# IceTTTb/NopeSAC

Hardware: AMD Instinct MI355X
Metric: image-pairs/sec (480x640, K=32 hyp) (higher is better)
Workload: dtype bf16; 1 GPU; configs/inference_mp3d.yaml, 32 synthetic 480x640 pairs/GPU/step, ResNet-50 + pyramids in bfloat16, head GEMMs bf16 operands with f32 accumulate / residual stream / LayerNorm / softmax, K=32 matched planes forced (m mean 32.0), nq=50; pairs_per_gpu=32, global_batch=32, K=32, parallelism=pair-sharded dp1, rccl_ranks=1, batches_in_flight_per_gpu=4, hip_graph=False, steps_per_all_gather=8, routing_entries_loaded=45, routing_entries_measured_now=0, nonfinite_outputs=0

## Files before the change

### include/nopesac_hip.h

```cpp
#ifndef NOPESAC_HIP_H
#define NOPESAC_HIP_H

#include <stdint.h>

#ifdef __cplusplus
extern "C" {
#endif

#define NPS_DT_F32 0
#define NPS_DT_BF16 1
#define NPS_DT_F32_BF16W 2
#define NPS_DT_FP8 3

#define NPS_ACT_NONE 0
#define NPS_ACT_RELU 1
#define NPS_ACT_LEAKY 2
#define NPS_ACT_SIGMOID 3
#define NPS_ACT_RES_AFTER 0x100
#define NPS_ACT_BIAS_BATCHED 0x200

#define NPS_E_ARG (-1)
#define NPS_E_UNSUPPORTED (-2)

int nopesac_version(void);
// ... 18 lines not shown

int nopesac_conv2d_nhwc_bfrag(const void* x, const void* w_frag, const float* scale, const float* bias, const void* residual,
                              void* y, int B, int H, int W, int Cin, int Cout, int KH, int KW, int stride, int pad,
                              int64_t x_cstride, int64_t y_cstride, int64_t r_cstride, int act, int out_dt, int variant,
                              void* stream);

int nopesac_conv2d_nhwc_p8(const void* x, const void* w, const float* scale, const float* bias, const void* residual, void* y,
                           int B, int H, int W, int Cin, int Cout, int KH, int KW, int stride, int pad,
                           int64_t x_cstride, int64_t y_cstride, int64_t r_cstride, int act, int out_dt, int variant, void* stream);

int64_t nopesac_conv2d_p8_sk_workspace_bytes(void);
int nopesac_conv2d_nhwc_p8_sk(const void* x, const void* w, const float* scale, const float* bias, const void* residual, void* y,
                              int B, int H, int W, int Cin, int Cout, int KH, int KW, int stride, int pad,
                              int64_t x_cstride, int64_t y_cstride, int64_t r_cstride, int act, int out_dt, int variant,
                              void* workspace, int64_t workspace_bytes, void* stream);

int nopesac_conv2d_nhwc_p8n(const void* x, const void* w, const float* scale, const float* bias, void* y, int B, int H, int W,
                            int Cin, int Cout, int KH, int KW, int stride, int pad, int64_t x_cstride, int64_t y_cstride, int act,
                            int variant, void* stream);
int nopesac_conv2d_nhwc_p8n_splitk(const void* x, const void* w, const float* scale, const float* bias, void* y, int B, int H, int W,
                                   int Cin, int Cout, int KH, int KW, int stride, int pad, int64_t x_cstride, int64_t y_cstride, int act,
                                   int variant, int splits, void* workspace, int64_t workspace_bytes, void* stream);

#define NOPESAC_MLP_MAX_IN 1280
#define NOPESAC_MLP_MAX_WIDTH 1024
#define NOPESAC_MLP_MAX_LAYERS 12
#define NOPESAC_MLP_RESTART 1
typedef struct nopesac_mlp_layer {
    const void* w;
    const float* bias;
    float* out;
    int64_t out_ld;
    int K, N, act, reserved;
} nopesac_mlp_layer;
typedef struct nopesac_mlp_chain {
    const float* x;
    int64_t x_ld;
    const float* xb;
    int64_t xb_ld;
    int x_width, xb_width, xb_rows_per, rows, n_layers, reserved;
    nopesac_mlp_layer layers[NOPESAC_MLP_MAX_LAYERS];
} nopesac_mlp_chain;
int nopesac_mlp_padded_k(int N, int K);
int64_t nopesac_mlp_packed_elems(int N, int K);
int nopesac_mlp_chain_bf16(const nopesac_mlp_chain* chain, void* stream);

int nopesac_conv2d_nhwc_fp8(const void* x, const void* w_frag8, const float* scale, const float* bias, const void* residual,
                            void* y, int B, int H, int W, int Cin, int Cout, int KH, int KW, int stride, int pad,
                            int64_t x_cstride, int64_t y_cstride, int64_t r_cstride, int act, int out_dt, int variant,
                            void* stream);

int nopesac_conv3x3_c64_bf16(const void* x, const void* w_frag, const float* scale, const float* bias, void* y, int B, int H, int W,
                             int act, void* stream);

int nopesac_conv3x3_halo_bf16(const void* x, const void* w_frag, const float* scale, const float* bias, void* y, int B, int H, int W,
                              int Cin, int Cout, int act, int tile, void* stream);

int nopesac_stem_fused_bf16(const void* x, const void* w, const float* scale, const float* bias, void* y,
                            int B, int H, int W, void* stream);
int nopesac_stem_fused_raw_bf16(const float* x_nchw, const float* mean, const float* std, const void* w, const float* scale,
                                const float* bias, void* y, int B, int H, int W, void* stream);
int nopesac_stem_fused_raw_shifted_bf16(const float* x_nchw, const float* pad3, const void* w_folded, const float* scale,
                                        const float* bias_folded, void* y, int B, int H, int W, void* stream);

int nopesac_bottleneck_tail_bf16(const void* b, const void* w3, const float* scale3, const float* bias3, const void* residual,
                                 const void* x2, const void* wsc, const float* scale_sc, const float* bias_sc, int B, int OH, int OW,
                                 int x2_H, int x2_W, int x2_stride, int C, int C4, int C2, void* y, const void* w1,
                                 const float* scale1, const float* bias1, int CN, void* o, void* stream);
int nopesac_bottleneck_tail_bf16_ex(const void* b, const void* w3, const float* scale3, const float* bias3, const void* residual,
                                    const void* x2, const void* wsc, const float* scale_sc, const float* bias_sc, int B, int OH, int OW,
                                    int x2_H, int x2_W, int x2_stride, int C, int C4, int C2, void* y, const void* w1,
                                    const float* scale1, const float* bias1, int CN, void* o, int o_dt, void* stream);

int nopesac_preprocess_nchw_to_nhwc(const float* x, void* y, const float* mean, const float* std,
                                    int B, int C, int H, int W, int Cpad, int out_dt, void* stream);

int nopesac_maxpool_nhwc(const void* x, void* y, int B, int H, int W, int C, int K, int stride, int pad,
                         int dt, void* stream);

int nopesac_upsample2x_bilinear_nhwc(const void* x, const void* addend, void* y, int B, int H, int W, int C,
                                     int act, int dt, void* stream);
int nopesac_upsample2x_nearest_add_nhwc(const void* x, const void* lateral, void* y, int B, int H, int W,
                                        int C, int dt, void* stream);

int nopesac_groupnorm_nhwc(const void* x, const float* gamma, const float* beta, void* y,
                           int B, int HW, int C, int G, float eps, int act, int dt, float* workspace, void* stream);

int nopesac_layernorm(const float* x, const float* res, const float* gamma, const float* beta,
                      float* y, const float* addend, int addend_rows, float* y2,
                      int rows, int D, float eps, void* stream);

int nopesac_layernorm_ex(const float* x, const float* res, const float* gamma, const float* beta,
                         float* y, const float* addend, int addend_rows, float* y2, void* y_bf16, void* y2_bf16,
                         int rows, int D, float eps, void* stream);

int nopesac_add_rows(const float* a, const float* b, float* out, int rows, int D, int b_rows, void* stream);

int nopesac_metric_rows(const float* trans, const float* rot, const int32_t* n1, const int32_t* n2, const int32_t* m,
                        const float* t_err, const float* r_err, const int32_t* nonfinite, int pair_idx0, float* rows, int B, void* stream);

int nopesac_concat_cols(const float* a, int Da, const float* b, int Db, float* out, int rows, void* stream);

int nopesac_add_rows_bf16(const float* a, const float* b, void* a_bf16, void* ab_bf16, int rows, int D, int b_rows, void* stream);

int nopesac_softmax_rows(const float* x, float* y, int rows, int D, void* stream);

// ... 234 lines not shown
```

### nopesac_amd/_lib.py

```python
from __future__ import annotations

import ctypes
import os
import re
from ctypes import c_char_p, c_float, c_int, c_int64, c_void_p

HERE = os.path.dirname(os.path.abspath(__file__))
LIB_PATH = os.path.join(HERE, "libnopesac_hip.so")
HEADER_PATH = os.path.join(os.path.dirname(HERE), "include", "nopesac_hip.h")

P, I, L, F = c_void_p, c_int, c_int64, c_float

SIGNATURES = {
    "nopesac_version": [],
    "nopesac_last_error": [],
    "nopesac_conv2d_nhwc": [P, P, P, P, P, P, I, I, I, I, I, I, I, I, I, L, L, L, L, I, I, I, P],
    "nopesac_conv2d_nhwc_bfrag": [P, P, P, P, P, P, I, I, I, I, I, I, I, I, I, L, L, L, I, I, I, P],
    "nopesac_conv2d_nhwc_p8": [P, P, P, P, P, P, I, I, I, I, I, I, I, I, I, L, L, L, I, I, I, P],
    "nopesac_conv2d_nhwc_p8_sk": [P, P, P, P, P, P, I, I, I, I, I, I, I, I, I, L, L, L, I, I, I, P, L, P],
    "nopesac_conv2d_p8_sk_workspace_bytes": [],
    "nopesac_conv2d_nhwc_p8n": [P, P, P, P, P, I, I, I, I, I, I, I, I, I, L, L, I, I, P],
    "nopesac_conv2d_nhwc_p8n_splitk": [P, P, P, P, P, I, I, I, I, I, I, I, I, I, L, L, I, I, I, P, L, P],
    "nopesac_conv2d_nhwc_ex": [P, P, P, P, P, P, I, I, I, I, I, I, I, I, I, L, L, L, L, I, I, I, I, P],
    "nopesac_stem_fused_bf16": [P, P, P, P, P, I, I, I, P],
    "nopesac_stem_fused_raw_bf16": [P, P, P, P, P, P, P, I, I, I, P],
    "nopesac_stem_fused_raw_shifted_bf16": [P, P, P, P, P, P, I, I, I, P],
    "nopesac_bottleneck_tail_bf16": [P] * 9 + [I] * 9 + [P] * 4 + [I, P, P],
    "nopesac_bottleneck_tail_bf16_ex": [P] * 9 + [I] * 9 + [P] * 4 + [I, P, I, P],
    "nopesac_conv2d_nhwc_fp8": [P, P, P, P, P, P, I, I, I, I, I, I, I, I, I, L, L, L, I, I, I, P],
    "nopesac_gnn_layer_bf16": [P, I, P, I, P, I, I, I, P, P] + [P] * 10 + [P],
    "nopesac_gnn_layer_bf16_pf": [P, I, P, I, P, I, I, I, P, P] + [P] * 10 + [P, I, P],
    "nopesac_encoder_tail_bf16": [P] * 13 + [I] + [P] * 3 + [I, P],
    "nopesac_resize_bilinear_u8": [P, I, I, I, P, I, I, P],
    "nopesac_resize_bilinear_u8_batch": [P, I, L, I, I, I, P, I, I, I, P],
    "nopesac_mask_head_bf16": [P] * 9 + [I] * 5 + [P],
    "nopesac_mask_operands": [P, I, P, P, I, I, I, P],
    "nopesac_decoder_tail_bf16": [P] * 13 + [I] + [P] * 4 + [I, P],
    "nopesac_transformer_tail_bf16": [P] * 13 + [I] + [P] * 4 + [I, I, P, P, P, I, P, P, P, I, I, P],
    "nopesac_transformer_tail_bf16_pf": [P] * 13 + [I] + [P] * 4 + [I, I, P, P, P, I, P, P, P, I, I, P, P, I, I, P],
    "nopesac_conv3x3_c64_bf16": [P, P, P, P, P, I, I, I, I, P],
    "nopesac_conv3x3_halo_bf16": [P, P, P, P, P, I, I, I, I, I, I, I, P],
    "nopesac_rle_labels": [P, P, P, P, P, I, I, I, I, P],
    "nopesac_rle_transitions": [P, P, P, P, P, I, I, I, P],
    "nopesac_rle_compress_host": [P, I, I, I, P, I, P],
    "nopesac_rle_compress_device": [P, P, P, I, I, I, P, P, P, P, P],
    "nopesac_rle_compress_device_capped": [P, P, P, I, I, I, P, P, P, L, P],
    "nopesac_decode_masks": [P, P, P, P, P, P, I, I, I, I, P],
    "nopesac_rle_compress_batch_host": [P, P, P, I, I, I, P, L, P, P],
    "nopesac_preprocess_nchw_to_nhwc": [P, P, P, P, I, I, I, I, I, I, P],
    "nopesac_maxpool_nhwc": [P, P, I, I, I, I, I, I, I, I, P],
    "nopesac_upsample2x_bilinear_nhwc": [P, P, P, I, I, I, I, I, I, P],
    "nopesac_upsample2x_nearest_add_nhwc": [P, P, P, I, I, I, I, I, P],
    "nopesac_groupnorm_nhwc": [P, P, P, P, I, I, I, I, F, I, I, P, P],
    "nopesac_layernorm": [P, P, P, P, P, P, I, P, I, I, F, P],
    "nopesac_layernorm_ex": [P, P, P, P, P, P, I, P, P, P, I, I, F, P],
    "nopesac_add_rows": [P, P, P, I, I, I, P],
    "nopesac_softmax_rows": [P, P, I, I, P],
    "nopesac_softmax_rows_pad": [P, P, I, I, I, I, P],
    "nopesac_add_rows_bf16": [P, P, P, P, I, I, I, P],
    "nopesac_concat_cols": [P, I, P, I, P, I, P],
    "nopesac_metric_rows": [P, P, P, P, P, P, P, P, I, P, I, P],
    "nopesac_attention_small": [P, L, P, L, P, L, P, L, I, I, I, I, F, P, P, P],
    "nopesac_attention_small_bf16": [P, L, P, L, P, L, P, L, I, I, I, I, F, P, P, P],
    "nopesac_attention_small_bf16io": [P, L, P, L, P, L, P, L, I, I, I, I, F, P, P, P],
    "nopesac_transpose_hw_rows": [P, P, I, I, I, I, P],
    "nopesac_postselect_planes": [P, P, P, P, I, I, I, I, I, I, I, F, F, F, P, P, P, P, P, P, P, P, P, P, P],
    "nopesac_postselect_planes_ex": [P, P, P, P, I, I, I, I, I, I, I, F, F, F, P, P, P, P, P, P, P, P, P, P, I, P],
    "nopesac_matcher_sinkhorn": [P, P, P, P, P, P, P, F, F, I, F, I, I, P, P, P],
    "nopesac_geo_sequence": [P, P, P, P, P, P, P, I, I, I, P, P, P, P, P, P],
    "nopesac_ransac_score_maps": [P, P, P, P, P, P, I, I, P, P, P, P, P, P, P, P, P, P],
    "nopesac_ransac_soft_vote": [P] * 21 + [I, I, I] + [P] * 6 + [P],
    "nopesac_plane_cam_ref_losses": [P] * 11 + [I, I, F, P, P],
    "nopesac_camera_pose_loss": [P, P, P, I, P, I, I, F, F, P, P],
    "nopesac_refilter_assignment": [P, P, P, P, P, P, P, I, I, P, P],
    "nopesac_tape_create": [P, ctypes.POINTER(c_void_p), P],
    "nopesac_tape_create_ex": [P, I, ctypes.POINTER(c_void_p), P],
    "nopesac_tape_replay": [P, P],
    "nopesac_tape_replay_on": [P, P, P, I],
    "nopesac_posenet_branch_tail_bf16": [P, P, P, P, P, P, P, I, I, I, I, P],
    "nopesac_tape_destroy": [P],
    "nopesac_lds_canary": [I, I, L, I, P, P, I, P],
    "nopesac_force_k_select": [P, I, P, P, P, I, I, I, I, P, P, P],
    "nopesac_normalize_rows": [P, P, I, I, I, P],
    "nopesac_count_nonfinite": [P, L, P, P],
    "nopesac_count_nonfinite_batch": [P, P, I, P, P],
    "nopesac_clock_probe": [P, L, P],
    "nopesac_u8_to_f32": [P, P, L, P],
    "nopesac_gather_bytes": [P, P, P, P, I, P, P],
    "nopesac_jpeg_huffman": [P, P, P, P, P, I, P, L, P, P, P],
    "nopesac_jpeg_huffman_parallel": [P, P, P, I, P, L, P, L, P, P, P, P, P, P, P, P],
    "nopesac_jpeg_prepare_scan": [P, L, I, P, L, P, P, P, L, P],
    "nopesac_jpeg_batch_scan_host": [P, I, I, I, P, P],
    "nopesac_jpeg_batch_fill_host": [P, P, P, P, P, P, P, P, P],
# ... 77 lines not shown
```

### nopesac_amd/build.py

```python
from __future__ import annotations

import hashlib
import os
import shutil
import subprocess
import sys
from concurrent.futures import ThreadPoolExecutor

HERE = os.path.dirname(os.path.abspath(__file__))
CSRC = os.path.join(HERE, "csrc")
LIB = os.path.join(HERE, "libnopesac_hip.so")
OBJ = os.path.join(CSRC, "_obj")
SOURCES = ["capi.hip", "conv_igemm.hip", "conv_p8.hip", "conv_p8n.hip", "stem.hip", "conv3x3_c64.hip", "conv3x3_halo.hip", "pwchain.hip", "gnn_layer.hip", "enc_tail.hip", "mask_head.hip", "resize.hip", "rle.hip", "elementwise.hip", "attention.hip", "postselect.hip", "matcher.hip",
           "ransac.hip", "refine_bwd.hip", "mlp_chain.hip", "tape.hip", "posenet_branch.hip", "jpeg.hip", "jpeg_host.hip", "png_host.hip"]
FLAGS = ["--offload-arch=gfx950", "-O3", "-std=c++17", "-fPIC", "-ffp-contract=off", "-Xclang", "-target-feature", "-Xclang", "-packed-fp32-ops"]
if os.environ.get("NOPESAC_ALLOW_PACKED_FP32"):
    FLAGS = FLAGS[:5]
EXTRA_FLAGS = {}
if os.environ.get("NOPESAC_HIPCC_EXTRA"):
    FLAGS = FLAGS + os.environ["NOPESAC_HIPCC_EXTRA"].split()


def _hipcc() -> str:
    for c in (os.environ.get("HIPCC"), shutil.which("hipcc"), "/opt/rocm/bin/hipcc"):
        if c and os.path.exists(c):
            return c
    raise RuntimeError("hipcc not found (need ROCm with gfx950 support)")


def _have_zlib(cc: str) -> bool:
    import tempfile
    with tempfile.TemporaryDirectory() as d:
        src = os.path.join(d, "z.cpp")
        with open(src, "w") as f:
            f.write("#include <zlib.h>\nint main() { z_stream s{}; return inflateInit(&s) == Z_OK ? inflateEnd(&s) : 1; }\n")
        r = subprocess.run([cc, "-x", "c++", src, "-o", os.path.join(d, "z"), "-lz"], capture_output=True, text=True)
        return r.returncode == 0


def _digest() -> str:
    h = hashlib.sha256((" ".join(FLAGS) + repr(sorted(EXTRA_FLAGS.items()))).encode())
    for name in sorted(os.listdir(CSRC)) + ["../../include/nopesac_hip.h"]:
        p = os.path.join(CSRC, name)
        if os.path.isfile(p) and (name.endswith((".hip", ".h"))):
            h.update(name.encode())
            h.update(open(p, "rb").read())
    return h.hexdigest()


def build(force: bool = False, verbose: bool = True) -> str:
    stamp = os.path.join(OBJ, "digest.txt")
    dig = _digest()
    if not force and os.path.exists(LIB) and os.path.exists(stamp) and open(stamp).read() == dig:
        return LIB
    os.makedirs(OBJ, exist_ok=True)
    cc = _hipcc()
    have_zlib = _have_zlib(cc)
    per_build = {"png_host.hip": ["-DNPS_HAVE_ZLIB=%d" % int(have_zlib)]}

    def compile_one(src):
        obj = os.path.join(OBJ, src.replace(".hip", ".o"))
        cmd = [cc, *FLAGS, *EXTRA_FLAGS.get(src, []), *per_build.get(src, []), "-c", os.path.join(CSRC, src), "-o", obj]
        r = subprocess.run(cmd, capture_output=True, text=True)
        if r.returncode != 0:
            raise RuntimeError("hipcc failed on %s:\n%s" % (src, r.stderr[-4000:]))
        return obj
# ... 17 lines not shown
```

### nopesac_amd/modeling/backbone.py

```python
from __future__ import annotations

import os

import torch

from .. import ops
from ..config import amd_options
from ..registry import BACKBONE_REGISTRY
from ..synth import RES_STAGES, state_dict_spec
from .params import DERIVED_EPOCH, ParamModule, conv_bn


class ShapeSpec:
    def __init__(self, channels=None, height=None, width=None, stride=None):
        self.channels, self.height, self.width, self.stride = channels, height, width, stride


class HipResNet50(ParamModule):
    size_divisibility = 0
    STEM_CIN_PAD = 4

    def __init__(self, cfg=None):
        spec = {k[len("backbone."):]: v for k, v in state_dict_spec(50).items() if k.startswith("backbone.")}
        super().__init__(spec)
        if cfg is not None:
            r = cfg.MODEL.RESNETS
            assert r.DEPTH == 50 and not r.STRIDE_IN_1X1 and r.NORM == "FrozenBN" and r.NUM_GROUPS == 1, \
                "only the ResNet-50 / FrozenBN / stride-in-3x3 configuration of configs/Base.yaml is implemented"
            self.out_features = list(r.OUT_FEATURES)
        else:
            self.out_features = ["res2", "res3", "res4", "res5"]
        self.fused_stem = True
        self.stem_folded_norm = os.environ.get("NOPESAC_STEM_FOLDED", "1") != "0"
        self.fused_tail = True
        self.halo_conv2 = not os.environ.get("NOPESAC_NO_HALO_CONV2")
        self.fp8_conv2 = bool(amd_options(cfg).BACKBONE_FP8) if cfg is not None else False
        self.act_scale: dict = {}
        self._calib: dict | None = None
        self._q8: dict = {}
        self.unfused_wide_tails = os.environ.get("NOPESAC_TAIL_RES4_FUSED", "0") != "1"
        self.rt4_res3_edges = os.environ.get("NOPESAC_RES3_EDGES_UNFUSED", "0") == "1"

    def output_shape(self):
        full = {"res2": ShapeSpec(256, stride=4), "res3": ShapeSpec(512, stride=8), "res4": ShapeSpec(1024, stride=16),
                "res5": ShapeSpec(2048, stride=32)}
        return {k: full[k] for k in self.out_features}

    def pack(self) -> dict:
        P = {"stem": conv_bn(self, "stem.conv1.weight", "stem.conv1.norm", 1e-5, cin_pad=self.STEM_CIN_PAD)}
        w = self.raw("stem.conv1.weight").float().permute(0, 2, 3, 1)
        w8 = w.new_zeros(64, 7, 8, 4)
        w8[:, :, :7, :3] = w
        P["stem_fused_w"] = w8.reshape(64, 224).to(torch.bfloat16).contiguous()
        cin = 64
        for name, n, cmid, cout in RES_STAGES:
            for i in range(n):
                p = f"{name}.{i}"
                for c in ("conv1", "conv2", "conv3") + (("shortcut",) if cin != cout else ()):
                    P[f"{p}.{c}"] = conv_bn(self, f"{p}.{c}.weight", f"{p}.{c}.norm", 1e-5)
                cin = cout
        return P

    def _apply(self, fn, *a, **k):
        self._q8 = {}
        return super()._apply(fn, *a, **k)

    def _load_from_state_dict(self, *a, **k):
        self._q8 = {}
        return super()._load_from_state_dict(*a, **k)

    def calibrate_fp8(self, x: torch.Tensor, headroom: float = 2.0) -> dict:
        was, self.fp8_conv2, self._calib = self.fp8_conv2, False, {}
        try:
            with torch.no_grad():
                self.forward(x)
            amax = {k: float(v) for k, v in self._calib.items()}
        finally:
            self.fp8_conv2, self._calib = was, None
        self.act_scale = {k: max(v, 1e-6) * headroom / ops.FP8_MAX for k, v in amax.items()}
        self._q8 = {}
        DERIVED_EPOCH[0] += 1
        return dict(self.act_scale)

    def _quant(self, p: str) -> dict:
        q = self._q8.get(p)
        if q is None:
            P = self.packed
            c1, c2 = P[p + ".conv1"], P[p + ".conv2"]
            xs = float(self.act_scale.get(p, 1.0))
            w8, wsc = ops.quantize_weights_fp8(c2.w(torch.float32))
            q = {"w8": w8, "s2": (c2.scale * wsc * xs).contiguous(), "s1": (c1.scale / xs).contiguous(), "b1": (c1.bias / xs).contiguous()}
            self._q8[p] = q
        return q

# ... 2 lines not shown
        dt = x.dtype if x is not None else torch.bfloat16
        assert x is not None or resume is not None or (raw is not None and self.fused_stem), "backbone: raw images need the fused bf16 stem"
        assert not self.fp8_conv2 or (dt == torch.bfloat16 and self.fused_tail), "MODEL.AMD.BACKBONE_FP8 needs MODEL.AMD.COMPUTE_DTYPE bfloat16"

        def cv(t, key, stride=1, pad=0, act=ops.ACT_RELU, residual=None):
            c = P[key]
            return ops.conv2d(t, c.w(dt), c.scale, c.bias, residual, stride=stride, pad=pad, act=act)

        stages = ["stem"] + [name for name, _, _, _ in RES_STAGES]
        skip_until = None
        if resume is not None:
            skip_until, x = resume
            dt = x.dtype
        elif x is None:
            if self.stem_folded_norm:
                key = ("stem_shift", raw[1].data_ptr(), raw[2].data_ptr())
                if key not in P:
                    P[key] = ops.fold_stem_normalisation(self.raw("stem.conv1.weight").float().permute(0, 2, 3, 1), P["stem"].scale,
                                                         P["stem"].bias, raw[1], raw[2])
                pad3, wsh, bsh = P[key]
                x = ops.stem_fused_raw_shifted(raw[0], pad3, wsh, P["stem"].scale, bsh)
            else:
                x = ops.stem_fused_raw(raw[0], raw[1], raw[2], P["stem_fused_w"], P["stem"].scale, P["stem"].bias)
        elif dt == torch.bfloat16 and self.fused_stem:
            x = ops.stem_fused(x, P["stem_fused_w"], P["stem"].scale, P["stem"].bias)
        else:
            x = cv(x, "stem", 2, 3)
            x = ops.maxpool(x, 3, 2, 1)
        if stop_after == "stem":
            return {"x": x}
        out = {}
        cin = 64
        fuse = dt == torch.bfloat16 and self.fused_tail
        blocks = [(name, i, n, cmid, cout) for name, n, cmid, cout in RES_STAGES for i in range(n)]
        a_pre = None
        for bi, (name, i, n, cmid, cout) in enumerate(blocks):
            if skip_until is not None and stages.index(name) <= stages.index(skip_until):
                cin = cout
                continue
            p = f"{name}.{i}"
            stride = 2 if (i == 0 and name != "res2") else 1
            proj = cin != cout
            fp8 = self.fp8_conv2 and cmid % 128 == 0
            if fp8:
                q = self._quant(p)
                if a_pre is None:
                    y = ops.conv2d(x, P[p + ".conv1"].w(dt), q["s1"], q["b1"], act=ops.ACT_RELU, out_dtype=torch.float8_e4m3fn)
                else:
                    y = a_pre
            else:
                y = a_pre if a_pre is not None else cv(x, p + ".conv1")
            if self._calib is not None:
                self._calib[p] = torch.maximum(self._calib.get(p, y.new_zeros((), dtype=torch.float32)), y.float().abs().amax())
            if fp8:
                c2 = P[p + ".conv2"]
                y = ops.conv2d_fp8(y, q["w8"], q["s2"], c2.bias, ksize=3, stride=stride, pad=1, act=ops.ACT_RELU)
            elif fuse and cmid == 64 and stride == 1 and self.halo_conv2:
                c2 = P[p + ".conv2"]
                y = ops.conv3x3_c64(y, c2.w(dt), c2.scale, c2.bias)
            else:
                y = cv(y, p + ".conv2", stride, 1)
            a_pre = None
            nxt = None
            if bi + 1 < len(blocks):
                nn_, ni = blocks[bi + 1][0], blocks[bi + 1][1]
                nxt = P[f"{nn_}.{ni}.conv1"]
            c3 = P[p + ".conv3"]
            cfg_next = (cmid, cout, nxt.cout if nxt is not None else 0, cin if proj else 0)
            cfg_solo = (cmid, cout, 0, cin if proj else 0)
            wide_unfused = self.unfused_wide_tails and cmid >= 256 and not self.fp8_conv2
            if fuse and not wide_unfused and (cfg_next in ops.BOTTLENECK_TAIL_CONFIGS or cfg_solo in ops.BOTTLENECK_TAIL_CONFIGS):
                use_next = cfg_next in ops.BOTTLENECK_TAIL_CONFIGS and nxt is not None
                kw = {}
                rt4_edges = self.rt4_res3_edges and cmid == 128 and not self.fp8_conv2
                if rt4_edges and use_next and nxt.cout > 128:
                    use_next = False
                if proj and rt4_edges:
                    kw.update(residual=cv(x, p + ".shortcut", stride, 0, ops.ACT_NONE))
                elif proj:
                    sc = P[p + ".shortcut"]
                    kw.update(x2=x, wsc=sc.wfrag(dt), ssc=sc.scale, bsc=sc.bias, stride=stride)
                else:
                    kw.update(residual=x)
                if use_next and self.fp8_conv2 and blocks[bi + 1][3] % 128 == 0:
                    qn = self._quant(f"{blocks[bi + 1][0]}.{blocks[bi + 1][1]}")
                    kw.update(w1=nxt.wfrag(dt), s1=qn["s1"], b1=qn["b1"], o_fp8=True)
                elif use_next:
                    kw.update(w1=nxt.wfrag(dt), s1=nxt.scale, b1=nxt.bias)
                x, a_pre = ops.bottleneck_tail(y, c3.wfrag(dt), c3.scale, c3.bias, **kw)
            else:
                sc = cv(x, p + ".shortcut", stride, 0, ops.ACT_NONE) if proj else x
                x = cv(y, p + ".conv3", residual=sc)
            cin = cout
            if i == n - 1 and name in self.out_features:
                out[name] = x
            if i == n - 1 and stop_after == name:
                return {"x": x}
        return out


@BACKBONE_REGISTRY.register()
def build_resnet_backbone(cfg, input_shape=None):
    return HipResNet50(cfg)


def build_backbone(cfg):
# ... 2 lines not shown
```

### nopesac_amd/ops.py

```python
from __future__ import annotations

from typing import Optional

import ctypes
import os

import torch

from . import _lib

F32, BF16 = 0, 1
ACT_NONE, ACT_RELU, ACT_LEAKY, ACT_SIGMOID = 0, 1, 2, 3
ACT_RES_AFTER = 0x100
ACT_BIAS_BATCHED = 0x200
FP8 = 3
_DT = {torch.float32: F32, torch.bfloat16: BF16, torch.float8_e4m3fn: FP8}


class OpsArgumentError(AssertionError, ValueError):
    """A wrapper's argument check failed.  Raised explicitly (not `assert`): the checks stay in force under `python -O`.
    (Subclasses AssertionError so that callers written against the first version keep working.)"""


def _require(cond, msg="argument check failed"):
# ... 404 lines not shown


FP8_MAX = 448.0


def quantize_weights_fp8(w: torch.Tensor):
    w2 = w.reshape(w.shape[0], -1).float()
    sc = w2.abs().amax(dim=1).clamp_min(1e-12) / FP8_MAX
    w8 = (w2 / sc[:, None]).clamp(-FP8_MAX, FP8_MAX).to(torch.float8_e4m3fn)
    return mfma_fragment_major_fp8(w8), sc.contiguous()


def conv2d_fp8(x: torch.Tensor, w8frag: torch.Tensor, scale: torch.Tensor, bias: torch.Tensor, *, ksize: int, stride=1, pad=0,
               act=ACT_NONE, out_dtype=torch.bfloat16, residual=None, variant: int = 0) -> torch.Tensor:
    _require(x.dtype == torch.float8_e4m3fn and w8frag.dtype == torch.float8_e4m3fn and x.is_contiguous() and w8frag.is_contiguous(), 'argument check failed: x.dtype == torch.float8_e4m3fn and w8frag.dtype == torch.float8_e4m3fn and x.is_contiguous() and w8frag.is_contiguous()')
    B, H, W, Cin = x.shape
    Cout = w8frag.shape[0]
    _require(w8frag.shape[1] == ksize * ksize * Cin, 'argument check failed: w8frag.shape[1] == ksize * ksize * Cin')
    _chk(scale, torch.float32); _chk(bias, torch.float32)
    OH = (H + 2 * pad - ksize) // stride + 1
    OW = (W + 2 * pad - ksize) // stride + 1
    out = torch.empty((B, OH, OW, Cout), device=x.device, dtype=out_dtype)
    if residual is not None:
        _chk(residual, out_dtype)
        _require(residual.shape == out.shape, 'argument check failed: residual.shape == out.shape')
    if not variant:
        variant = 3 if Cin % 128 == 0 else 32
    rc = _L().nopesac_conv2d_nhwc_fp8(_p(x), _p(w8frag), _p(scale), _p(bias), _p(residual), _p(out), B, H, W, Cin, Cout, ksize, ksize,
                                      stride, pad, Cin, Cout, Cout if residual is not None else 0, act, _DT[out_dtype], variant, _stream())
    _lib.check(rc, "nopesac_conv2d_nhwc_fp8")
    return out


def bottleneck_tail(b, w3, s3, b3, *, residual=None, x2=None, wsc=None, ssc=None, bsc=None, stride=1, w1=None, s1=None, b1=None,
                    o_fp8: bool = False):
    _chk(b, torch.bfloat16); _chk(w3, torch.bfloat16)
    B, OH, OW, C = b.shape
    C4 = w3.shape[0]
    CN = 0 if w1 is None else w1.shape[0]
    C2 = 0 if x2 is None else x2.shape[3]
    _require((C, C4, CN, C2) in BOTTLENECK_TAIL_CONFIGS, (C, C4, CN, C2))
    y = torch.empty((B, OH, OW, C4), device=b.device, dtype=torch.bfloat16)
    o = torch.empty((B, OH, OW, CN), device=b.device, dtype=torch.float8_e4m3fn if o_fp8 else torch.bfloat16) if CN else None
    if residual is not None:
        _chk(residual, torch.bfloat16)
        _require(residual.shape == y.shape, 'argument check failed: residual.shape == y.shape')
    if x2 is not None:
        _chk(x2, torch.bfloat16); _chk(wsc, torch.bfloat16)
    H2, W2 = (x2.shape[1], x2.shape[2]) if x2 is not None else (0, 0)
    rc = _L().nopesac_bottleneck_tail_bf16_ex(_p(b), _p(w3), _p(s3), _p(b3), _p(residual), _p(x2), _p(wsc), _p(ssc), _p(bsc), B, OH, OW,
                                              H2, W2, stride, C, C4, C2, _p(y), _p(w1), _p(s1), _p(b1), CN, _p(o),
                                              FP8 if o_fp8 else BF16, _stream())
    _lib.check(rc, "nopesac_bottleneck_tail_bf16_ex")
    return y, o


def maxpool(x: torch.Tensor, k: int, stride: int, pad: int) -> torch.Tensor:
    _chk(x)
    B, H, W, C = x.shape
    OH, OW = (H + 2 * pad - k) // stride + 1, (W + 2 * pad - k) // stride + 1
    y = torch.empty((B, OH, OW, C), device=x.device, dtype=x.dtype)
    _lib.check(_L().nopesac_maxpool_nhwc(_p(x), _p(y), B, H, W, C, k, stride, pad, _DT[x.dtype], _stream()), "nopesac_maxpool_nhwc")
    return y


def upsample2x_bilinear(x: torch.Tensor, addend=None, act=ACT_NONE) -> torch.Tensor:
    _chk(x)
    B, H, W, C = x.shape
    y = torch.empty((B, 2 * H, 2 * W, C), device=x.device, dtype=x.dtype)
    if addend is not None:
        _chk(addend, x.dtype)
        _require(addend.shape == y.shape, 'argument check failed: addend.shape == y.shape')
    _lib.check(_L().nopesac_upsample2x_bilinear_nhwc(_p(x), _p(addend), _p(y), B, H, W, C, act, _DT[x.dtype], _stream()),
               "nopesac_upsample2x_bilinear_nhwc")
    return y


def upsample2x_nearest_add(x: torch.Tensor, lateral: torch.Tensor) -> torch.Tensor:
    _chk(x); _chk(lateral, x.dtype)
    B, H, W, C = x.shape
    _require(lateral.shape == (B, 2 * H, 2 * W, C), 'argument check failed: lateral.shape == (B, 2 * H, 2 * W, C)')
    y = torch.empty_like(lateral)
    _lib.check(_L().nopesac_upsample2x_nearest_add_nhwc(_p(x), _p(lateral), _p(y), B, H, W, C, _DT[x.dtype], _stream()),
               "nopesac_upsample2x_nearest_add_nhwc")
    return y


def groupnorm(x: torch.Tensor, gamma, beta, groups: int, eps: float, act=ACT_NONE) -> torch.Tensor:
    _chk(x)
    B, H, W, C = x.shape
    y = torch.empty_like(x)
    ws = torch.empty(B * 16 * groups * 2, device=x.device, dtype=torch.float32)
    _lib.check(_L().nopesac_groupnorm_nhwc(_p(x), _p(_chk(gamma, torch.float32)), _p(_chk(beta, torch.float32)), _p(y), B, H * W, C,
                                           groups, eps, act, _DT[x.dtype], _p(ws), _stream()), "nopesac_groupnorm_nhwc")
    return y


def layernorm(x: torch.Tensor, gamma, beta, res=None, addend=None, eps=1e-5):
    _chk(x, torch.float32)
    D = x.shape[-1]
    rows = x.numel() // D
    y = torch.empty_like(x)
    y2 = torch.empty_like(x) if addend is not None else None
    if res is not None:
        _chk(res, torch.float32)
        _require(res.shape == x.shape, 'argument check failed: res.shape == x.shape')
# ... 622 lines not shown
```

Measured before the change: 4076 pairs/s.

## Fuse res2 bottleneck conv2, conv3, residual and next conv1 into one kernel

```diff
diff --git a/include/nopesac_hip.h b/include/nopesac_hip.h
--- a/include/nopesac_hip.h
+++ b/include/nopesac_hip.h
@@ -94,6 +94,10 @@
 
 int nopesac_conv3x3_c64_bf16(const void* x, const void* w_frag, const float* scale, const float* bias, void* y, int B, int H, int W,
                              int act, void* stream);
+
+int nopesac_bottleneck_block_bf16(const void* a, const void* x, const void* w2_frag, const float* scale2, const float* bias2,
+                                  const void* w3, const float* scale3, const float* bias3, const void* w1, const float* scale1,
+                                  const float* bias1, void* y, void* o, int B, int H, int W, int C, int C4, int CN, void* stream);
 
 int nopesac_conv3x3_halo_bf16(const void* x, const void* w_frag, const float* scale, const float* bias, void* y, int B, int H, int W,
                               int Cin, int Cout, int act, int tile, void* stream);
diff --git a/nopesac_amd/_lib.py b/nopesac_amd/_lib.py
--- a/nopesac_amd/_lib.py
+++ b/nopesac_amd/_lib.py
@@ -39,6 +39,7 @@
     "nopesac_transformer_tail_bf16": [P] * 13 + [I] + [P] * 4 + [I, I, P, P, P, I, P, P, P, I, I, P],
     "nopesac_transformer_tail_bf16_pf": [P] * 13 + [I] + [P] * 4 + [I, I, P, P, P, I, P, P, P, I, I, P, P, I, I, P],
     "nopesac_conv3x3_c64_bf16": [P, P, P, P, P, I, I, I, I, P],
+    "nopesac_bottleneck_block_bf16": [P] * 13 + [I] * 6 + [P],
     "nopesac_conv3x3_halo_bf16": [P, P, P, P, P, I, I, I, I, I, I, I, P],
     "nopesac_rle_labels": [P, P, P, P, P, I, I, I, I, P],
     "nopesac_rle_transitions": [P, P, P, P, P, I, I, I, P],
diff --git a/nopesac_amd/build.py b/nopesac_amd/build.py
--- a/nopesac_amd/build.py
+++ b/nopesac_amd/build.py
@@ -11,7 +11,7 @@
 CSRC = os.path.join(HERE, "csrc")
 LIB = os.path.join(HERE, "libnopesac_hip.so")
 OBJ = os.path.join(CSRC, "_obj")
-SOURCES = ["capi.hip", "conv_igemm.hip", "conv_p8.hip", "conv_p8n.hip", "stem.hip", "conv3x3_c64.hip", "conv3x3_halo.hip", "pwchain.hip", "gnn_layer.hip", "enc_tail.hip", "mask_head.hip", "resize.hip", "rle.hip", "elementwise.hip", "attention.hip", "postselect.hip", "matcher.hip",
+SOURCES = ["capi.hip", "conv_igemm.hip", "conv_p8.hip", "conv_p8n.hip", "stem.hip", "conv3x3_c64.hip", "conv3x3_halo.hip", "pwchain.hip", "block_fused.hip", "gnn_layer.hip", "enc_tail.hip", "mask_head.hip", "resize.hip", "rle.hip", "elementwise.hip", "attention.hip", "postselect.hip", "matcher.hip",
            "ransac.hip", "refine_bwd.hip", "mlp_chain.hip", "tape.hip", "posenet_branch.hip", "jpeg.hip", "jpeg_host.hip", "png_host.hip"]
 FLAGS = ["--offload-arch=gfx950", "-O3", "-std=c++17", "-fPIC", "-ffp-contract=off", "-Xclang", "-target-feature", "-Xclang", "-packed-fp32-ops"]
 if os.environ.get("NOPESAC_ALLOW_PACKED_FP32"):
diff --git a/nopesac_amd/csrc/block_fused.hip b/nopesac_amd/csrc/block_fused.hip
--- /dev/null
+++ b/nopesac_amd/csrc/block_fused.hip
@@ -0,0 +1,352 @@
+#include "common.h"
+
+namespace nps {
+
+namespace bf {
+
+typedef float f32x16 __attribute__((ext_vector_type(16)));
+typedef float f32x4 __attribute__((ext_vector_type(4)));
+typedef __bf16 bf16x8 __attribute__((ext_vector_type(8)));
+typedef unsigned short us8 __attribute__((ext_vector_type(8)));
+typedef unsigned short us4 __attribute__((ext_vector_type(4)));
+
+constexpr int C = 64, T = 16, HT = T + 2;
+constexpr int PXB = (C + 8) * 2;
+constexpr int ROWB = ((HT * PXB + 255) / 256) * 256;
+constexpr int HALO_BYTES = HT * ROWB;
+constexpr int KS = 9 * C / 16;
+constexpr int RING = 16;
+constexpr int BM = 128, CH = 128, A_LD = C + 8, Y_LD = CH + 8;
+constexpr int KF1 = C / 16, KF2 = CH / 16;
+constexpr int RCH = BM * (CH / 8) / 256;
+constexpr int B_BYTES = 2 * BM * A_LD * 2;
+constexpr int Y_OFF = B_BYTES, Y_BYTES = BM * Y_LD * 2;
+
+template <int C4>
+struct Lds {
+    static constexpr int S3_OFF = Y_OFF + Y_BYTES;
+    static constexpr int S2_OFF = S3_OFF + 2 * C4 * 4;
+    static constexpr int BYTES = S2_OFF + 2 * C * 4;
+    static_assert(HALO_BYTES <= S3_OFF, "the bn vectors lie outside the halo (they are written before it dies)");
+    static_assert(2 * BYTES <= 160 * 1024 && BYTES <= 80 * 1024, "two workgroups per CU");
+};
+
+}
+
+template <int C4, int CN>
+__global__ __launch_bounds__(256, 2) void bottleneck_block_kernel(const bf16_t* __restrict__ a, const bf16_t* __restrict__ x,
+                                                                  const bf16_t* __restrict__ w2frag, const float* __restrict__ s2,
+                                                                  const float* __restrict__ b2, const bf16_t* __restrict__ w3,
+                                                                  const float* __restrict__ s3, const float* __restrict__ b3,
+                                                                  const bf16_t* __restrict__ w1, const float* __restrict__ s1,
+                                                                  const float* __restrict__ b1, bf16_t* __restrict__ y,
+                                                                  bf16_t* __restrict__ o, int H, int W) {
+    using namespace bf;
+    typedef Lds<C4> L;
+    constexpr int NCH = C4 / CH;
+    constexpr int NR2 = CN >= 128 ? 4 : 2;
+    constexpr int O_LD = CN + 8;
+    static_assert(C4 % CH == 0 && (CN == 0 || CN == 64 || CN == 128), "block shapes");
+    static_assert(CN == 0 || BM * O_LD <= BM * Y_LD, "the a' staging tile aliases the y chunk");
+    extern __shared__ __attribute__((aligned(16))) unsigned char bf_smem[];
+    unsigned char* lds = bf_smem;
+    float* S3 = reinterpret_cast<float*>(bf_smem + L::S3_OFF);
+    float* B3 = S3 + C4;
+    float* sb2 = reinterpret_cast<float*>(bf_smem + L::S2_OFF);
+    bf16_t* Y = reinterpret_cast<bf16_t*>(bf_smem + Y_OFF);
+    bf16_t* O = Y;
+
+    const int tid = threadIdx.x, lane = tid & 63, l31 = lane & 31, half = lane >> 5;
+    const int wave = __builtin_amdgcn_readfirstlane(tid >> 6);
+    const int bimg = blockIdx.z, y0 = blockIdx.y * T, x0 = blockIdx.x * T;
+    const float sb_v = (tid & 64 ? b2 : s2)[tid & 63];
+    constexpr int NSB = (C4 / 4 + 256 - 1) / 256;
+    f32x4 sbv[NSB][2];
+#pragma unroll
+    for (int it = 0; it < NSB; ++it) {
+        const int i = tid + it * 256 < C4 / 4 ? tid + it * 256 : C4 / 4 - 1;
+        sbv[it][0] = *reinterpret_cast<const f32x4*>(s3 + 4 * i);
+        sbv[it][1] = *reinterpret_cast<const f32x4*>(b3 + 4 * i);
+    }
+    const int nt = wave & 1, rt0 = (wave >> 1) * 4;
+    const bf16_t* wp = w2frag + ((long long)nt * KS * 64 + lane) * 8;
+    bf16x8 ring[RING];
+#pragma unroll
+    for (int s = 0; s < RING; ++s) ring[s] = *reinterpret_cast<const bf16x8*>(wp + s * 512);
+    const bf16_t* ab = a + (long long)bimg * H * W * C;
+    {
+        constexpr int NIT = (HT * HT * 8 + 255) / 256;
+        us8 hv[NIT];
+#pragma unroll
+        for (int it = 0; it < NIT; ++it) {
+            const int i = tid + it * 256;
+            const int px = i >> 3, ch = (i & 7) * 8;
+            const int iy = y0 - 1 + px / HT, ix = x0 - 1 + px % HT;
+            const int iyc = iy < 0 ? 0 : (iy >= H ? H - 1 : iy), ixc = ix < 0 ? 0 : (ix >= W ? W - 1 : ix);
+            hv[it] = *reinterpret_cast<const us8*>(ab + ((long long)iyc * W + ixc) * C + ch);
+        }
+#pragma unroll
+        for (int it = 0; it < NIT; ++it) {
+            const int i = tid + it * 256;
+            const int px = i >> 3;
+            const int iy = y0 - 1 + px / HT, ix = x0 - 1 + px % HT;
+            const bool in = (unsigned)iy < (unsigned)H && (unsigned)ix < (unsigned)W;
+            if (i < HT * HT * 8) *reinterpret_cast<us8*>(lds + (px / HT) * ROWB + (px % HT) * PXB + (i & 7) * 16) = in ? hv[it] : us8{};
+        }
+    }
+    if (tid < 128) sb2[tid] = sb_v;
+#pragma unroll
+    for (int it = 0; it < NSB; ++it) {
+        const int i = tid + it * 256;
+        if (i < C4 / 4) {
+            *reinterpret_cast<f32x4*>(S3 + 4 * i) = sbv[it][0];
+            *reinterpret_cast<f32x4*>(B3 + 4 * i) = sbv[it][1];
+        }
+    }
+    __syncthreads();
+
+    {
+        f32x16 acc[4];
+#pragma unroll
+        for (int r = 0; r < 4; ++r)
+#pragma unroll
+            for (int e = 0; e < 16; ++e) acc[r][e] = 0.f;
+        int a_off[4];
+#pragma unroll
+        for (int r = 0; r < 4; ++r) {
+            const int ty = 2 * (rt0 + r) + (l31 >> 4), tx = l31 & 15;
+            a_off[r] = ty * ROWB + tx * PXB + half * 16;
+        }
+#pragma unroll
+        for (int ks = 0; ks < KS; ++ks) {
+            const int tap = ks >> 2, kk = ks & 3, kh = tap / 3, kw = tap % 3;
+            const int t_off = kh * ROWB + kw * PXB + kk * 32;
+#pragma unroll
+            for (int r = 0; r < 4; ++r) {
+                const bf16x8 af = *reinterpret_cast<const bf16x8*>(lds + a_off[r] + t_off);
+                acc[r] = __builtin_amdgcn_mfma_f32_32x32x16_bf16(ring[ks % RING], af, acc[r], 0, 0, 0);
+            }
+            if (ks + RING < KS) ring[ks % RING] = *reinterpret_cast<const bf16x8*>(wp + (ks + RING) * 512);
+            if ((ks & 3) == 3) __builtin_amdgcn_sched_barrier(0);
+        }
+        __syncthreads();
+        float ev[64];
+#pragma unroll
+        for (int q = 0; q < 4; ++q) {
+            const int n = nt * 32 + 8 * q + 4 * half;
+            const f32x4 s = *reinterpret_cast<const f32x4*>(sb2 + n), bb = *reinterpret_cast<const f32x4*>(sb2 + 64 + n);
+#pragma unroll
+            for (int r = 0; r < 4; ++r)
+#pragma unroll
+                for (int e = 0; e < 4; ++e) {
+                    float v = acc[r][4 * q + e] * s[e];
+                    v += bb[e];
+                    ev[(q * 4 + r) * 4 + e] = v;
+                }
+        }
+        apply_act_n<64>(ev, NPS_ACT_RELU);
+#pragma unroll
+        for (int q = 0; q < 4; ++q) {
+            const int n = nt * 32 + 8 * q + 4 * half;
+#pragma unroll
+            for (int r = 0; r < 4; ++r) {
+                us4 v;
+#pragma unroll
+                for (int e = 0; e < 4; ++e) v[e] = f32_to_bf16(ev[(q * 4 + r) * 4 + e]);
+                *reinterpret_cast<us4*>(lds + ((rt0 + r) * 32 + l31) * PXB + n * 2) = v;
+            }
+        }
+    }
+
+    const int wl = half * 32 + 16 * ((l31 >> 2) & 1) + 4 * (l31 >> 3) + (l31 & 3);
+    const int nt2 = CN >= 128 ? wave : (wave & 1);
+    const int r2 = CN >= 128 ? 0 : 2 * (wave >> 1);
+    bf16x8 wa[KF1], wb[CN ? KF2 : 1];
+    auto load_wa = [&](int c) {
+        const bf16_t* w = w3 + ((long long)((c * (CH / 32) + wave) * KF1) * 64 + wl) * 8;
+#pragma unroll
+        for (int kk = 0; kk < KF1; ++kk) wa[kk] = *reinterpret_cast<const bf16x8*>(w + kk * 512);
+    };
+    auto load_wb = [&](int c) {
+        if constexpr (CN > 0) {
+            const bf16_t* w = w1 + ((long long)(nt2 * (C4 / 16) + c * KF2) * 64 + wl) * 8;
+#pragma unroll
+            for (int kk = 0; kk < KF2; ++kk) wb[kk] = *reinterpret_cast<const bf16x8*>(w + kk * 512);
+        }
+    };
+    const long long img = (long long)bimg * H * W;
+    const char* res_img = reinterpret_cast<const char*>(x + img * C4);
+    char* y_img = reinterpret_cast<char*>(y + img * C4);
+    const int trow = tid >> 4, tcol = (tid & 15) * 16;
+    const int srow = (tid >> 5) * 2 + (((lane >> 2) ^ (lane >> 3) ^ (lane >> 4)) & 1);
+    const int rx = x0 + trow < W ? x0 + trow : W - 1;
+    const bool sx_in = x0 + srow < W;
+    auto res_off = [&](int h, int i) -> unsigned {
+        const int yy = y0 + 8 * h + i;
+        return (unsigned)(((yy < H ? yy : H - 1) * W + rx) * (C4 * 2) + tcol);
+    };
+    us8 rres[RCH];
+    auto fetch_res = [&](int h, int c) {
+#pragma unroll
+        for (int i = 0; i < RCH; ++i) rres[i] = *reinterpret_cast<const us8*>(res_img + c * (CH * 2) + res_off(h, i));
+    };
+    auto park_res = [&]() {
+#pragma unroll
+        for (int i = 0; i < RCH; ++i) *reinterpret_cast<us8*>(Y + (trow + 16 * i) * Y_LD + (tid & 15) * 8) = rres[i];
+    };
+    fetch_res(0, 0);
+    load_wa(0);
+    park_res();
+    __syncthreads();
+
+#pragma unroll
+    for (int h = 0; h < 2; ++h) {
+        if (h == 1) {
+            if (y0 + 8 >= H) break;
+            park_res();
+            __syncthreads();
+        }
+        const bf16_t* A1 = reinterpret_cast<const bf16_t*>(lds) + h * BM * A_LD;
+        f32x16 acc2[CN ? NR2 : 1];
+#pragma unroll
+        for (int r = 0; r < (CN ? NR2 : 1); ++r)
+#pragma unroll
+            for (int e = 0; e < 16; ++e) acc2[r][e] = 0.f;
+#pragma unroll
+        for (int c = 0; c < NCH; ++c) {
+            load_wb(c);
+            if (c + 1 < NCH) fetch_res(h, c + 1);
+            else if (h == 0) fetch_res(1, 0);
+#pragma unroll
+            for (int rp = 0; rp < 2; ++rp) {
+                f32x16 acc[2];
+#pragma unroll
+                for (int r = 0; r < 2; ++r)
+#pragma unroll
+                    for (int e = 0; e < 16; ++e) acc[r][e] = 0.f;
+#pragma unroll
+                for (int kk = 0; kk < KF1; ++kk)
+#pragma unroll
+                    for (int r = 0; r < 2; ++r) {
+                        const bf16x8 af = *reinterpret_cast<const bf16x8*>(A1 + ((2 * rp + r) * 32 + l31) * A_LD + kk * 16 + half * 8);
+                        acc[r] = __builtin_amdgcn_mfma_f32_32x32x16_bf16(wa[kk], af, acc[r], 0, 0, 0);
+                        if (r == 1 && (kk & 1)) __builtin_amdgcn_sched_barrier(0);
+                    }
+#pragma unroll
+                for (int qq = 0; qq < 2; ++qq) {
+                    const int nl = wave * 32 + 16 * half + 8 * qq, n = c * CH + nl;
+                    f32x4 sc3[2], bc3[2];
+#pragma unroll
+                    for (int j = 0; j < 2; ++j) { sc3[j] = *reinterpret_cast<const f32x4*>(S3 + n + 4 * j); bc3[j] = *reinterpret_cast<const f32x4*>(B3 + n + 4 * j); }
+#pragma unroll
+                    for (int r = 0; r < 2; ++r) {
+                        bf16_t* yp = Y + ((2 * rp + r) * 32 + l31) * Y_LD + nl;
+                        const us8 r8 = *reinterpret_cast<const us8*>(yp);
+                        us8 o8;
+#pragma unroll
+                        for (int j = 0; j < 2; ++j)
+#pragma unroll
+                            for (int e = 0; e < 4; ++e) {
+                                float v = acc[r][4 * (2 * qq + j) + e] * sc3[j][e];
+                                v += bc3[j][e];
+                                v += bf16_to_f32(r8[4 * j + e]);
+                                o8[4 * j + e] = f32_to_bf16(v > 0.f ? v : 0.f);
+                            }
+                        *reinterpret_cast<us8*>(yp) = o8;
+                    }
+                }
+                __builtin_amdgcn_sched_barrier(0);
+            }
+            __syncthreads();
+#pragma unroll
+            for (int i = 0; i < RCH; ++i) {
+                const us8 v = *reinterpret_cast<const us8*>(Y + (srow + 16 * i) * Y_LD + (tid & 15) * 8);
+                const int yy = y0 + 8 * h + i;
+                if (sx_in && yy < H)
+                    *reinterpret_cast<us8*>(y_img + c * (CH * 2) + (unsigned)((yy * W + x0 + srow) * (C4 * 2) + tcol)) = v;
+            }
+            __builtin_amdgcn_sched_barrier(0);
+            if (c + 1 < NCH) load_wa(c + 1);
+            else if (h == 0) load_wa(0);
+            if constexpr (CN > 0) {
+#pragma unroll
+                for (int kk = 0; kk < KF2; ++kk)
+#pragma unroll
+                    for (int r = 0; r < NR2; ++r) {
+                        const bf16x8 af = *reinterpret_cast<const bf16x8*>(Y + ((r2 + r) * 32 + l31) * Y_LD + kk * 16 + half * 8);
+                        acc2[r] = __builtin_amdgcn_mfma_f32_32x32x16_bf16(wb[kk], af, acc2[r], 0, 0, 0);
+                        if (r == NR2 - 1 && (kk & 1)) __builtin_amdgcn_sched_barrier(0);
+                    }
+            }
+            __syncthreads();
+            if (c + 1 < NCH) {
+                park_res();
+                __syncthreads();
+            }
+        }
+        if constexpr (CN > 0) {
+#pragma unroll
+            for (int qq = 0; qq < 2; ++qq) {
+                const int n = nt2 * 32 + 16 * half + 8 * qq;
+                f32x4 sc1[2], bc1[2];
+#pragma unroll
+                for (int j = 0; j < 2; ++j) { sc1[j] = *reinterpret_cast<const f32x4*>(s1 + n + 4 * j); bc1[j] = *reinterpret_cast<const f32x4*>(b1 + n + 4 * j); }
+#pragma unroll
+                for (int r = 0; r < NR2; ++r) {
+                    us8 o8;
+#pragma unroll
+                    for (int j = 0; j < 2; ++j)
+#pragma unroll
+                        for (int e = 0; e < 4; ++e) {
+                            float v = acc2[r][4 * (2 * qq + j) + e] * sc1[j][e];
+                            v += bc1[j][e];
+                            o8[4 * j + e] = f32_to_bf16(v > 0.f ? v : 0.f);
+                        }
+                    *reinterpret_cast<us8*>(O + ((r2 + r) * 32 + l31) * O_LD + n) = o8;
+                }
+            }
+            __syncthreads();
+            constexpr int CPR = CN / 8, RPI = 256 / CPR;
+            static_assert(BM * CPR % 256 == 0, "a' tile chunking");
+            const int orow = tid / CPR, ocol = tid % CPR;
+            char* o_img = reinterpret_cast<char*>(o + img * CN);
+#pragma unroll
+            for (int i = 0; i < BM * CPR / 256; ++i) {
+                const int row = orow + i * RPI;
+                const int yy = y0 + 8 * h + (row >> 4), xx = x0 + (row & 15);
+                const us8 v = *reinterpret_cast<const us8*>(O + row * O_LD + ocol * 8);
+                if (yy < H && xx < W) *reinterpret_cast<us8*>(o_img + (unsigned)((yy * W + xx) * (CN * 2) + ocol * 16)) = v;
+            }
+            if (h == 0) __syncthreads();
+        }
+    }
+}
+
+}
+
+extern "C" int nopesac_bottleneck_block_bf16(const void* a, const void* x, const void* w2_frag, const float* scale2, const float* bias2,
+                                             const void* w3, const float* scale3, const float* bias3, const void* w1, const float* scale1,
+                                             const float* bias1, void* y, void* o, int B, int H, int W, int C, int C4, int CN, void* stream) {
+    using namespace nps;
+    NPS_CHECK_ARG(a && x && w2_frag && scale2 && bias2 && w3 && scale3 && bias3 && y, "bottleneck_block: null pointer");
+    NPS_CHECK_ARG(B > 0 && H > 0 && W > 0, "bottleneck_block: bad shape B=%d H=%d W=%d", B, H, W);
+    NPS_CHECK_ARG(C == 64 && C4 == 256 && (CN == 64 || CN == 128), "bottleneck_block: unsupported channels C=%d C4=%d CN=%d", C, C4, CN);
+    NPS_CHECK_ARG(w1 && scale1 && bias1 && o, "bottleneck_block: null next-conv1 pointer");
+    NPS_CHECK_ARG((long long)H * W * C4 * 2 < (1ll << 31), "bottleneck_block: image too large (32-bit in-image offsets)");
+    const void* ptrs[] = {a, x, w2_frag, scale2, bias2, w3, scale3, bias3, w1, scale1, bias1, y, o};
+    for (const void* q : ptrs) NPS_CHECK_ARG(((uintptr_t)q & 15) == 0, "bottleneck_block: pointers must be 16-byte aligned");
+    const dim3 grid((W + bf::T - 1) / bf::T, (H + bf::T - 1) / bf::T, B);
+    constexpr int lds = bf::Lds<256>::BYTES;
+    hipStream_t st = (hipStream_t)stream;
+#define BF_LAUNCH(cn)                                                                                                                      \
+    if (CN == cn) {                                                                                                                        \
+        NPS_ENSURE_LDS(lds, bottleneck_block_kernel<256, cn>);                                                                             \
+        hipLaunchKernelGGL((bottleneck_block_kernel<256, cn>), grid, dim3(256), lds, st, (const bf16_t*)a, (const bf16_t*)x,              \
+                           (const bf16_t*)w2_frag, scale2, bias2, (const bf16_t*)w3, scale3, bias3, (const bf16_t*)w1, scale1, bias1,      \
+                           (bf16_t*)y, (bf16_t*)o, H, W);                                                                                  \
+        NPS_LAUNCH_RET();                                                                                                                  \
+    }
+    BF_LAUNCH(64) BF_LAUNCH(128)
+#undef BF_LAUNCH
+    return NPS_E_ARG;
+}
diff --git a/nopesac_amd/modeling/backbone.py b/nopesac_amd/modeling/backbone.py
--- a/nopesac_amd/modeling/backbone.py
+++ b/nopesac_amd/modeling/backbone.py
@@ -40,6 +40,9 @@
         self._q8: dict = {}
         self.unfused_wide_tails = os.environ.get("NOPESAC_TAIL_RES4_FUSED", "0") != "1"
         self.rt4_res3_edges = os.environ.get("NOPESAC_RES3_EDGES_UNFUSED", "0") == "1"
+        self.fused_blocks = set(os.environ.get("NOPESAC_BLOCK_FUSED", "res2.1,res2.2").split(",")) - {""}
+        if os.environ.get("NOPESAC_BLOCK_UNFUSED"):
+            self.fused_blocks = set()
 
     def output_shape(self):
         full = {"res2": ShapeSpec(256, stride=4), "res3": ShapeSpec(512, stride=8), "res4": ShapeSpec(1024, stride=16),
@@ -148,6 +151,18 @@
                 y = a_pre if a_pre is not None else cv(x, p + ".conv1")
             if self._calib is not None:
                 self._calib[p] = torch.maximum(self._calib.get(p, y.new_zeros((), dtype=torch.float32)), y.float().abs().amax())
+            if (fuse and not self.fp8_conv2 and self.halo_conv2 and p in self.fused_blocks and stride == 1 and not proj
+                    and bi + 1 < len(blocks)
+                    and (cmid, cout, P[f"{blocks[bi + 1][0]}.{blocks[bi + 1][1]}.conv1"].cout) in ops.BOTTLENECK_BLOCK_CONFIGS):
+                c2, c3, nxt = P[p + ".conv2"], P[p + ".conv3"], P[f"{blocks[bi + 1][0]}.{blocks[bi + 1][1]}.conv1"]
+                x, a_pre = ops.bottleneck_block(y, x, c2.w(dt), c2.scale, c2.bias, c3.wfrag(dt), c3.scale, c3.bias,
+                                                nxt.wfrag(dt), nxt.scale, nxt.bias)
+                cin = cout
+                if i == n - 1 and name in self.out_features:
+                    out[name] = x
+                if i == n - 1 and stop_after == name:
+                    return {"x": x}
+                continue
             if fp8:
                 c2 = P[p + ".conv2"]
                 y = ops.conv2d_fp8(y, q["w8"], q["s2"], c2.bias, ksize=3, stride=stride, pad=1, act=ops.ACT_RELU)
diff --git a/nopesac_amd/ops.py b/nopesac_amd/ops.py
--- a/nopesac_amd/ops.py
+++ b/nopesac_amd/ops.py
@@ -480,6 +480,27 @@
                                               H2, W2, stride, C, C4, C2, _p(y), _p(w1), _p(s1), _p(b1), CN, _p(o),
                                               FP8 if o_fp8 else BF16, _stream())
     _lib.check(rc, "nopesac_bottleneck_tail_bf16_ex")
+    return y, o
+
+
+BOTTLENECK_BLOCK_CONFIGS = {(64, 256, 64), (64, 256, 128)}
+
+
+def bottleneck_block(a, x, w2, s2, b2, w3, s3, b3, w1=None, s1=None, b1=None):
+    _chk(a, torch.bfloat16); _chk(x, torch.bfloat16); _chk(w2, torch.bfloat16); _chk(w3, torch.bfloat16)
+    _chk(s2, torch.float32); _chk(b2, torch.float32); _chk(s3, torch.float32); _chk(b3, torch.float32)
+    _require(w1 is not None, "bottleneck_block: the fused block needs the next block's conv1 (w1, s1, b1)")
+    _chk(w1, torch.bfloat16); _chk(s1, torch.float32); _chk(b1, torch.float32)
+    B, H, W, C = a.shape
+    C4, CN = w3.shape[0], w1.shape[0]
+    _require((C, C4, CN) in BOTTLENECK_BLOCK_CONFIGS, (C, C4, CN))
+    _require(tuple(w2.shape) == (C, 3, 3, C), 'argument check failed: tuple(w2.shape) == (C, 3, 3, C)')
+    _require(tuple(x.shape) == (B, H, W, C4), 'argument check failed: tuple(x.shape) == (B, H, W, C4)')
+    y = torch.empty((B, H, W, C4), device=a.device, dtype=torch.bfloat16)
+    o = torch.empty((B, H, W, CN), device=a.device, dtype=torch.bfloat16)
+    rc = _L().nopesac_bottleneck_block_bf16(_p(a), _p(x), _p(_frag_weights(w2)), _p(s2), _p(b2), _p(w3), _p(s3), _p(b3), _p(w1), _p(s1),
+                                            _p(b1), _p(y), _p(o), B, H, W, C, C4, CN, _stream())
+    _lib.check(rc, "nopesac_bottleneck_block_bf16")
     return y, o
 
 
```

Measured after the change: 4113 pairs/s, median of 6. No clear change (+0.9%).
